# openclimatefix/graph_weather

Measured on AMD Instinct MI355X. Metric: forward forecasts/sec (1° grid, 102→78 feat), higher is better.
Workload: dtype f32; 1 GPU; c2: GraphWeatherForecaster 1deg grid (64800 nodes), 102->78 feat, batch=2 on rank 0, fp32, mesh res 2 (5882 nodes), random-init weights; global_batch=2, parallelism=batch-sharded x1, no collective in forward

## Files before the change

### graph_weather_amd/_lib.py

```python
from __future__ import annotations

import ctypes
import os
import subprocess
from ctypes import POINTER, Structure, c_char_p, c_float, c_int, c_int32, c_int64, c_size_t, c_void_p

_HERE = os.path.dirname(os.path.abspath(__file__))
CSRC = os.path.join(_HERE, "csrc")
LIB_PATH = os.path.join(CSRC, "libgw_amd.so")
HIPCC_FLAGS = ["--offload-arch=gfx950", "-O3", "-std=c++17", "-munsafe-fp-atomics", "-shared", "-fPIC"]

ABI_VERSION = 19
DTYPE_F32, DTYPE_BF16, DTYPE_BF16X3 = 0, 1, 2
LAYOUT_ROWS_F32, LAYOUT_EDGE_TILES_BF16, LAYOUT_ROWS_F16, LAYOUT_ROWS_BF16K = 0, 1, 2, 3
EDGE_DETERMINISTIC, EDGE_SEGMENT_TILES, EDGE_AGG_BF16K, EDGE_SEGMENT_SPLIT = 1, 2, 4, 8

EXPORTS = [
    "gw_version", "gw_last_error", "gw_debug_timestamps", "gw_packed_floats", "gw_pack_linear", "gw_packed_bytes_bf16",
    "gw_pack_linear_bf16", "gw_packed_bytes_bf16x3", "gw_pack_linear_bf16x3", "gw_padded_n", "gw_pad_vector", "gw_pack_many", "gw_mlp_chain_backward", "gw_mlp_chain_backward_bf16x3", "gw_mlp_ln_chain_backward",
    "gw_mlp_forward", "gw_mlp_post_forward", "gw_project_forward", "gw_edge_update_forward", "gw_edge_update_workspace_bytes", "gw_edge_tiles_bytes",
    "gw_edge_rows_to_tiles", "gw_node_update_forward", "gw_node_update_row_split_groups", "gw_node_update_head_forward",
    "gw_normalized_mse_forward", "gw_gemm_f32", "gw_relu_backward", "gw_layernorm_backward", "gw_gather_rows",
    "gw_segment_sum_rows", "gw_normalized_mse_backward", "gw_adamw_step", "gw_nudging_forward", "gw_nudging_backward",
    "gw_linear_forward", "gw_linear_gather_forward", "gw_layernorm_forward", "gw_add_rows", "gw_gather_rows_wide", "gw_segment_sum_rows_wide",
    "gw_constraint_workspace_bytes", "gw_constraint_forward", "gw_constraint_backward",
    "gw_thermal_conv_forward", "gw_thermal_conv_wgrad_workspace_bytes", "gw_thermal_conv_wgrad", "gw_thermal_colsum_workspace_bytes",
    "gw_thermal_colsum", "gw_thermal_groupnorm_workspace_bytes", "gw_thermal_groupnorm_forward", "gw_thermal_groupnorm_backward",
    "gw_thermal_maxpool_forward", "gw_thermal_maxpool_backward", "gw_thermal_resize_forward", "gw_thermal_resize_backward",
    "gw_thermal_rows",
    "gw_amse_mmax", "gw_amse_dft_rows", "gw_amse_legendre_floats", "gw_amse_coeff_floats", "gw_amse_workspace_bytes",
    "gw_amse_forward", "gw_amse_backward",
    "gw_modulate_workspace_bytes", "gw_sdl_forward", "gw_sdl_backward", "gw_film_forward", "gw_film_backward",
    "gw_attention_forward", "gw_attention_backward", "gw_knn_interpolate_forward", "gw_knn_interpolate_backward",
    "gw_gelu_forward", "gw_gelu_backward",
    "gw_attention_axial_forward", "gw_attention_axial_backward",
    "gw_patch_workspace_bytes", "gw_patch_embed_forward", "gw_patch_embed_backward", "gw_patch_expand_forward",
    "gw_patch_expand_backward",
    "gw_attention_masked_forward", "gw_attention_masked_backward",
    "gw_earth_loss_workspace_bytes", "gw_earth_loss_forward", "gw_earth_loss_backward",
    "gw_token_mean_forward", "gw_token_mean_backward", "gw_relu_forward", "gw_row_scale",
    "gw_conv3d_workspace_bytes", "gw_conv3d_forward", "gw_conv3d_backward",
    "gw_gemm_tn_ordered_workspace_bytes", "gw_gemm_tn_ordered", "gw_layernorm_backward_ordered_workspace_bytes",
    "gw_layernorm_backward_ordered",
]

GEMM_NN, GEMM_TN, GEMM_TN_BF16X3 = 0, 1, 2


class GwOperand(Structure):
    _fields_ = [("ptr", c_void_p), ("index", c_void_p), ("rows_per_batch", c_int32), ("ld", c_int32), ("k", c_int32),
                ("projected", c_int32), ("layout", c_int32)]


class GwMlpWeights(Structure):
    _fields_ = [("w1", c_void_p * 3), ("b1", c_void_p), ("w_mid", c_void_p), ("b_mid", c_void_p), ("w_out", c_void_p),
                ("b_out", c_void_p), ("ln_gamma", c_void_p), ("ln_beta", c_void_p), ("hidden", c_int32),
                ("n_mid", c_int32), ("n_out", c_int32), ("weight_dtype", c_int32), ("ln_width", c_int32), ("k_in", c_int32),
                ("out_rows", c_int32)]


PACK_MAX_ITEMS = 16


class GwPackItem(Structure):
    _fields_ = [("w", c_void_p), ("stride_f", c_int64), ("stride_k", c_int64), ("n_out", c_int32), ("kseg", c_int32),
                ("rows", c_int32), ("reserved", c_int32), ("out", c_void_p)]
# ... 96 lines not shown
    L.gw_pad_vector.argtypes = [c_void_p, c_int, c_void_p, c_void_p]
    L.gw_mlp_chain_backward.restype = c_int
    L.gw_mlp_chain_backward.argtypes = [c_int64, c_void_p, c_int32, c_int32, POINTER(c_void_p), POINTER(c_void_p), POINTER(c_void_p),
                                        c_int32, POINTER(c_void_p), POINTER(c_void_p), c_void_p]
    L.gw_mlp_chain_backward_bf16x3.restype = c_int
    L.gw_mlp_chain_backward_bf16x3.argtypes = L.gw_mlp_chain_backward.argtypes
    L.gw_mlp_ln_chain_backward.restype = c_int
    L.gw_mlp_ln_chain_backward.argtypes = [c_int32, c_int64, c_void_p, c_int32, c_void_p, c_int32, c_int32, c_void_p, c_int32,
                                           c_void_p, c_void_p, c_void_p, c_void_p, c_void_p,
                                           c_int32, POINTER(c_void_p), POINTER(c_void_p), POINTER(c_void_p), c_void_p,
                                           c_int32, POINTER(c_void_p), POINTER(c_void_p), POINTER(c_void_p), c_int32, ctypes.c_uint32, c_void_p]
    L.gw_pack_many.restype = c_int
    L.gw_pack_many.argtypes = [c_int32, c_int32, POINTER(GwPackItem), c_int32, POINTER(GwPadItem), c_void_p]
    L.gw_mlp_forward.restype = c_int
    L.gw_mlp_forward.argtypes = [c_int64, c_int32, POINTER(GwOperand), POINTER(GwMlpWeights), POINTER(GwOperand),
                                 c_void_p, c_int32, POINTER(GwActivationSave), c_void_p]
    L.gw_mlp_post_forward.restype = c_int
    L.gw_mlp_post_forward.argtypes = [c_int64, c_int32, POINTER(GwOperand), POINTER(GwMlpWeights), c_void_p, c_int32, c_int32,
                                      POINTER(c_void_p), POINTER(c_void_p), c_int32, c_void_p]
    L.gw_edge_update_forward.restype = c_int
    L.gw_edge_update_forward.argtypes = [c_int32, c_int32, c_void_p, c_void_p, POINTER(GwOperand), POINTER(GwOperand),
                                         POINTER(GwOperand), POINTER(GwOperand), POINTER(GwMlpWeights), c_void_p, c_int32, c_void_p,
                                         c_int32, POINTER(GwActivationSave), c_void_p, c_size_t, c_int32, c_void_p]
    L.gw_edge_tiles_bytes.restype = c_size_t
    L.gw_edge_tiles_bytes.argtypes = [c_int32, c_int32]
    L.gw_edge_rows_to_tiles.restype = c_int
    L.gw_edge_rows_to_tiles.argtypes = [c_int32, c_int32, c_void_p, c_int32, c_int32, c_void_p, c_void_p]
    L.gw_edge_update_workspace_bytes.restype = c_size_t
    L.gw_edge_update_workspace_bytes.argtypes = [c_int32, c_int32, POINTER(GwOperand), POINTER(GwOperand), POINTER(GwOperand),
                                                 POINTER(GwMlpWeights), c_int32]
    L.gw_node_update_forward.restype = c_int
    L.gw_node_update_forward.argtypes = [c_int64, c_int32, POINTER(GwOperand), POINTER(GwOperand), POINTER(GwOperand),
                                         POINTER(GwMlpWeights), c_void_p, c_int32, POINTER(GwActivationSave), c_int32,
                                         POINTER(c_void_p), POINTER(c_void_p), c_int32, c_void_p, c_void_p]
    L.gw_node_update_row_split_groups.restype = c_int
    L.gw_node_update_row_split_groups.argtypes = [c_int64]
    L.gw_node_update_head_forward.restype = c_int
    L.gw_node_update_head_forward.argtypes = [c_int64, c_int32, POINTER(GwOperand), POINTER(GwOperand), POINTER(GwMlpWeights),
                                              POINTER(GwMlpWeights), POINTER(GwOperand), c_void_p, c_int32, c_void_p]
    L.gw_project_forward.restype = c_int
    L.gw_project_forward.argtypes = [c_int64, c_int32, POINTER(GwOperand), c_int32, POINTER(c_void_p), POINTER(c_void_p),
                                     c_int32, c_int32, c_int32, c_void_p, c_void_p, c_void_p]
    L.gw_normalized_mse_forward.restype = c_int
    L.gw_normalized_mse_forward.argtypes = [c_void_p, c_void_p, c_void_p, c_int32, c_void_p, c_int32, c_int32, c_int32, c_int32,
                                            c_void_p, c_void_p]
    L.gw_gemm_f32.restype = c_int
# ... 194 lines not shown
```

### graph_weather_amd/autograd.py

```python
from __future__ import annotations

from typing import List, Optional, Sequence, Tuple

import torch

from . import _lib, ops
from .ops import Operand, SavedActivations


def _st(t: torch.Tensor) -> int:
    return torch.cuda.current_stream(t.device).cuda_stream


def _L():
    return _lib.lib()


def gemm_nn(a: torch.Tensor, b: torch.Tensor, n: int, b_col0: int = 0, out: Optional[torch.Tensor] = None) -> torch.Tensor:
    m, k = int(a.shape[0]), int(a.shape[1])
    if out is None:
        out = torch.empty((m, n), dtype=torch.float32, device=a.device)
    _lib.check(_L().gw_gemm_f32(_lib.GEMM_NN, m, n, k, a.data_ptr(), int(a.stride(0)), b.data_ptr() + 4 * b_col0,
                                int(b.stride(0)), out.data_ptr(), int(out.stride(0)), None, _st(a)), "gw_gemm_f32 NN")
    return out
# ... 274 lines not shown
        grads[0] = gW0
        dx = fo[fan[0]] if fan else None
        dres = None
        if ctx.has_res and ctx.needs_input_grad[2]:
            n_out = int(dy.shape[1])
            if res.shape[1] == n_out:
                dres = dy
            else:
                dres = torch.zeros_like(res)
                dres[:, :n_out] = dy
        return (None, dx, dres, None, None, None, None, *grads)


def mlp_rows(mlp, x2: torch.Tensor, n_rows: int, rows_per_batch: int, residual_op: Optional[Operand] = None) -> torch.Tensor:
    params = mlp.native_params()
    if residual_op is None:
        return MLPRowsFunction.apply(mlp, x2, None, 0, 0, n_rows, rows_per_batch, *params)
    return MLPRowsFunction.apply(mlp, x2, residual_op.tensor, residual_op.rows_per_batch, residual_op.k, n_rows, rows_per_batch,
                                 *params)


class RecomputeFunction(torch.autograd.Function):

    @staticmethod
    def forward(ctx, fn, n_in, params, *tensors):
        ctx.fn, ctx.n_in, ctx.params = fn, n_in, params
        ctx.save_for_backward(*tensors[:n_in])
        with torch.no_grad():
            outs = fn(*tensors[:n_in])
        return tuple(outs)

    @staticmethod
    def backward(ctx, *douts):
        n_in, params = ctx.n_in, ctx.params
        ins = [t.detach().requires_grad_(bool(need)) for t, need in zip(ctx.saved_tensors, ctx.needs_input_grad[3:3 + n_in])]
        with torch.enable_grad():
            outs = ctx.fn(*ins)
        pairs = [(o, d) for o, d in zip(outs, douts) if d is not None and o.requires_grad]
        wanted = [t for t in ins if t.requires_grad] + [p for p in params if p.requires_grad]
        got = iter(torch.autograd.grad([o for o, _ in pairs], wanted, [d for _, d in pairs], allow_unused=True)) if pairs and wanted \
            else iter(())
        g_in = [next(got, None) if t.requires_grad else None for t in ins]
        g_par = [next(got, None) if p.requires_grad else None for p in params]
        return (None, None, None, *g_in, *g_par)


def recompute(fn, inputs: Sequence[torch.Tensor], module) -> Tuple[torch.Tensor, ...]:
    mods = module if isinstance(module, (list, tuple)) else [module]
    params = [p for m in mods for p in m.parameters()]
    if not torch.is_grad_enabled() or not (any(p.requires_grad for p in params) or any(t.requires_grad for t in inputs)):
        return tuple(fn(*inputs))
    return RecomputeFunction.apply(fn, len(inputs), params, *inputs, *params)


def _input_grad_joined(mlp, d: torch.Tensor, W: torch.Tensor, lo: int, hi: int, addend: Optional[torch.Tensor]) -> torch.Tensor:
    if addend is None:
        return input_grad(mlp, 0, d, W, lo, hi)
    pt = _packed_transposed(mlp, 0, W, lo, hi) if (d.shape[1] == 256 and d.stride(0) % 4 == 0 and d.shape[0] > 0) else None
    if (pt is not None and addend.shape == d.shape and addend.stride(1) == 1 and addend.stride(0) % 4 == 0 and addend.stride(0) >= 256
            and addend.dtype == torch.float32):
        out = torch.empty((int(d.shape[0]), 256), dtype=torch.float32, device=d.device)
        chain_backward(d, [], [(pt, out)], fan_add=[addend])
        return out
    return input_grad(mlp, 0, d, W, lo, hi).add_(addend)


class ProjectFunction(torch.autograd.Function):
# ... 264 lines not shown
```

### graph_weather_amd/layers.py

```python
from __future__ import annotations

from typing import List, Optional, Tuple

import torch
from torch import nn

from . import autograd as ag
from . import ops
from . import routes
from . import wide
from .autograd import OperandSpec
from .graphs import ForecastGraphs, GraphPlan, build_forecast_graphs
from .ops import BF16X3, Operand, PackedMLP
from .thermalizer import ThermalizerLayer

_NORMS = ["LayerNorm", "GraphNorm", "InstanceNorm", "BatchNorm", "MessageNorm"]


def _ver(t: torch.Tensor) -> int:
    return -1 if t.is_inference() else t._version


def _version_key(params) -> tuple:
    return tuple((p.data_ptr(), _ver(p), p.device) for p in params)
# ... 600 lines not shown

    def mesh_embedding(self) -> torch.Tensor:
        ps = list(self.node_encoder.parameters()) + [self.h3_nodes]
        return self._cached("mesh", ps, lambda: self.node_encoder.table(self.h3_nodes if _autograd_on(self) else self.h3_nodes.detach()))

    def encoder_edge_embedding(self, plan: GraphPlan) -> torch.Tensor:
        return self._cached("enc_e", list(self.edge_encoder.parameters()), lambda: self.edge_encoder.table(plan.edge_attr))

    def latent_edge_embedding(self, plan: GraphPlan) -> torch.Tensor:
        return self._cached("lat_e", list(self.latent_edge_encoder.parameters()),
                            lambda: self.latent_edge_encoder.table(plan.edge_attr))

    def encode(self, features: torch.Tensor, post_w=None):
        if features.dim() != 3 or features.shape[1] != self.num_latlons:
            raise RuntimeError("features must be [B, %d, input_dim]" % self.num_latlons)
        B, G, F = (int(s) for s in features.shape)
        if wide.encoder_is_wide(self):
            return wide.encode(self, features)
        feats = features.contiguous().reshape(B * G, F)
        enc_plan, _ = self._plans(features.device)
        team = self.team_path(features)
        x3 = self.split_path(features)
        ne = self.node_encoder
        fused_ps = None
        if ((team and ne.compute_dtype == torch.bfloat16) or (x3 and ne.compute_dtype == BF16X3)) and not ne._layout()[4] \
                and 32 < ne.native_k() <= 128:
            pm_e0 = self.graph_processor.blocks[0].edge_model.edge_mlp.packed()
            k = ne.native_k()
            x2 = feats if k <= F else torch.nn.functional.pad(feats, (0, k - F))
            fused_ps = ops.mlp_post_forward(ne.packed(), Operand(x2, G, k), B * G, G, [pm_e0.w1[0]], post_half=team)[1][0]
            xg = None
        else:
            xg = ne.run(feats, B * G, G)
        xm = self.mesh_embedding()
        e = self.encoder_edge_embedding(enc_plan)
        blk = self.graph_processor.blocks[0]
        _check_native_dims(*self.graph_processor._dims)
        pd_xm, pe, px_xm, e = self._static_projections(blk, xm, e)
        x_src, e_res = Feed(xg, G, "raw"), e
        seg = None
        if team or x3:
            pm_e = blk.edge_model.edge_mlp.packed()
            if fused_ps is None:
                fused_ps = ops.project_forward([pm_e.w1[0]], Operand(xg, G, 256), B * G, G, out_half=team)[0]
            x_src = Feed(fused_ps, G, "proj")
            px_xm = self._team_node_product(blk, enc_plan, e, px_xm)
            e_res = None
        if team:
            seg = enc_plan.seg_tiles(split=True)
            if seg is not None:
                pe = self._cached("enc_pe_pad", list(self.parameters()), lambda: seg.pad_rows(pe))
        if post_w is not None:
            x, _, posts, agg0 = blk.run(B, enc_plan, x_src, Feed(pd_xm, 0, "proj"), Feed(pe, 0, "proj"), e_res, 0,
                                        Feed(px_xm, 0, "proj"), xm, 0, False, features.device, tag="encoder_edge",
                                        post_w=post_w, post_zero=True, seg=seg)
            return x, posts, agg0
        x, _ = blk.run(B, enc_plan, x_src, Feed(pd_xm, 0, "proj"), Feed(pe, 0, "proj"), e_res, 0,
                       Feed(px_xm, 0, "proj"), xm, 0, False, features.device, tag="encoder_edge", seg=seg)
        return x

    def team_path(self, features: Optional[torch.Tensor] = None) -> bool:
        return self._block_route(features) == routes.BLOCK_TEAM

    def _block_route(self, features: Optional[torch.Tensor] = None) -> str:
        blk = self.graph_processor.blocks[0]
        mlp_e, mlp_n = blk.edge_model.edge_mlp, blk.node_model.node_mlp
        is_wide = wide.encoder_is_wide(self)
        auto = False if is_wide else _autograd_on(self, features)
        if is_wide or auto:
            return routes.BLOCK_ROWS
        return routes.block_route(_form(mlp_e), mlp_n.compute_dtype, self.graphs.enc_plan.num_edges, False, False,
                                  bool(blk.deterministic))

    def split_path(self, features: Optional[torch.Tensor] = None) -> bool:
        return self._block_route(features) == routes.BLOCK_SPLIT

    def _team_node_product(self, blk, plan: GraphPlan, e: torch.Tensor, px_xm: torch.Tensor) -> torch.Tensor:
        def make():
            pm_n = blk.node_model.node_mlp.packed()
            n_e = int(e.shape[0])
            e_sum = ag.segment_sum_rows(e, n_e, 1, 1, plan.n_dst, plan.dst_ptr(), None)
            pa = ops.project_forward([pm_n.w1[1]], Operand(e_sum, plan.n_dst, 256), plan.n_dst, plan.n_dst)[0]
# ... 352 lines not shown
```

### graph_weather_amd/ops.py

```python
from __future__ import annotations

from dataclasses import dataclass
from typing import List, Optional, Sequence, Tuple

import torch

from . import _lib
from ._lib import GwActivationSave, GwMlpWeights, GwOperand


class KernelTimer:

    def __init__(self, tags):
        self.tags = set(tags)
        self.events = {t: [] for t in self.tags}
        self.units = {t: [] for t in self.tags}

    def start(self, tag):
        if tag not in self.tags:
            return None
        ev = (torch.cuda.Event(enable_timing=True), torch.cuda.Event(enable_timing=True))
        ev[0].record()
        return ev

    def stop(self, tag, ev, units: int = 1):
        if ev is not None:
            ev[1].record()
            self.events[tag].append(ev)
            self.units[tag].append(int(units))

    def mean_units(self, tag) -> float:
        u = self.units[tag]
        return sum(u) / max(1, len(u))

    def mean_ms(self, tag) -> float:
        evs = self.events[tag]
        return sum(a.elapsed_time(b) for a, b in evs) / max(1, len(evs))


TIMER: Optional[KernelTimer] = None

EDGE_STREAM = True
"""float32 inference: the decoder's edge update runs without the per-edge residual on the decoder-form kernel of
csrc/gw_edge_stream.hip (the segment sums of the batch-shared edge embedding enter the node update as a cached product).
``False`` forces the per-edge residual route on ``edge_kernel`` (csrc/gw_edge.hip).  Read on every ``decode``."""


def _stream(t: torch.Tensor) -> int:
    return torch.cuda.current_stream(t.device).cuda_stream


class _NoGuard:
    def __enter__(self):
        return None

    def __exit__(self, *exc):
        return False


_NO_GUARD = _NoGuard()


def on_device_of(t: torch.Tensor):
    idx = t.device.index
    if idx is None or idx == torch.cuda.current_device():
        return _NO_GUARD
    return torch.cuda.device(idx)

# ... 281 lines not shown
            _require(e_out, "e_out")
    n_edges = int(src.shape[0])
    wc = pm.c((x_src.k > 0 and not x_src.projected, x_dst.k > 0 and not x_dst.projected, e_in.k > 0 and not e_in.projected))
    xs, xd, ei = x_src.c(), x_dst.c(), e_in.c()
    flags = _lib.EDGE_DETERMINISTIC if deterministic else 0
    if segment_tiles:
        flags |= _lib.EDGE_SEGMENT_TILES | (_lib.EDGE_AGG_BF16K if agg_bf16 else 0) | (_lib.EDGE_SEGMENT_SPLIT if segment_split else 0)
    ws, ws_bytes = None, 0
    if save is None:
        ws_bytes = int(_lib.lib().gw_edge_update_workspace_bytes(batch, n_edges, xs, xd, ei, wc, flags))
        if ws_bytes:
            ws = torch.empty(ws_bytes, dtype=torch.uint8, device=agg.device)
    ev = TIMER.start(tag) if TIMER is not None else None
    with on_device_of(agg):
        _lib.check(_lib.lib().gw_edge_update_forward(batch, n_edges, src.data_ptr(), dst.data_ptr(), xs, xd, ei,
                                                     e_res.c(), wc, None if e_out is None else e_out.data_ptr(), e_out_layout,
                                                     agg.data_ptr(), n_dst, None if save is None else save.c(),
                                                     None if ws is None else ws.data_ptr(), ws_bytes, flags, _stream(agg)),
                   "gw_edge_update_forward")
    if ev is not None:
        TIMER.stop(tag, ev, batch)


def node_update_forward(pm: PackedMLP, n_rows: int, rows_per_batch: int, x: Operand, x_res: Operand, agg: Operand,
                        out: Optional[torch.Tensor] = None, save: Optional[SavedActivations] = None,
                        post_w: Optional[Sequence[torch.Tensor]] = None, zero_rows: Optional[torch.Tensor] = None,
                        post_half: bool = False):
    import ctypes

    dev = agg.tensor.device
    if out is None:
        out = torch.empty((n_rows, pm.n_out), dtype=torch.float32, device=dev)
    _require(out, "out")
    wc = pm.c((x.k > 0 and not x.projected, True, False))
    n_post = 0 if post_w is None else len(post_w)
    outs, wp, op = [], None, None
    if n_post:
        outs = [torch.empty((n_rows, 256), dtype=torch.float16 if post_half else torch.float32, device=dev) for _ in range(n_post)]
        wp = (ctypes.c_void_p * n_post)(*[w_.data_ptr() for w_ in post_w])
        op = (ctypes.c_void_p * n_post)(*[o_.data_ptr() for o_ in outs])
    with on_device_of(out):
        _lib.check(_lib.lib().gw_node_update_forward(n_rows, rows_per_batch, x.c(), x_res.c(), agg.c(), wc, out.data_ptr(),
                                                     int(out.stride(0)), None if save is None else save.c(), n_post, wp, op,
                                                     _lib.LAYOUT_ROWS_F16 if (post_half and n_post) else _lib.LAYOUT_ROWS_F32,
                                                     None if zero_rows is None else zero_rows.data_ptr(), _stream(out)),
                   "gw_node_update_forward")
# ... 200 lines not shown
```

### graph_weather_amd/routes.py

```python
from __future__ import annotations

from dataclasses import dataclass
from typing import Optional, Sequence, Tuple

import torch

BF16X3 = "bf16x3"



@dataclass(frozen=True)
class MlpForm:

    dtype: object
    n_mid: int
    ln_width: int
    has_norm: bool

    @staticmethod
    def of(mlp, packed=None) -> "MlpForm":
        pm = mlp.packed() if packed is None else packed
        return MlpForm(mlp.compute_dtype, int(pm.n_mid), int(pm.ln_width), pm.gamma is not None)


# ... 31 lines not shown

BLOCK_ROWS = "rows"
BLOCK_TEAM = "team"
BLOCK_SPLIT = "split"


def block_route(edge: MlpForm, node_dtype, n_edges: int, wide: bool, autograd: bool, deterministic: bool) -> str:
    if wide or autograd or n_edges <= 0:
        return BLOCK_ROWS
    if edge.dtype == BF16X3 and node_dtype == BF16X3:
        return BLOCK_SPLIT
    if edge.dtype == torch.bfloat16 and node_dtype == torch.bfloat16 and not deterministic and resident_bf16(edge, n_edges):
        return BLOCK_TEAM
    return BLOCK_ROWS


def decoder_stream(edge: MlpForm, node_dtype, n_edges: int, wide: bool, autograd: bool, deterministic: bool, enabled: bool) -> bool:
    if not enabled or wide or autograd or deterministic or n_edges <= 0:
        return False
    return (edge.dtype == torch.float32 and node_dtype == torch.float32 and edge.n_mid == 1 and edge.ln_width == 0
            and edge.has_norm)




def stack_on_segment_tiles(blocks: Sequence[Tuple[MlpForm, object, bool]], n_edges: int, max_slots: Optional[int]) -> bool:
    if len(blocks) == 0 or n_edges <= 0 or max_slots is None or max_slots > 16:
        return False
    return all(resident_bf16(e, n_edges) and nd == torch.bfloat16 and not det for e, nd, det in blocks)


def segment_route_allowed(train: bool, want_edges: bool, lo: int, shared: bool) -> bool:
    return (not train) and (not want_edges) and lo == 0 and shared


def mesh_streams(streams_attr: int, edge_dtypes: Sequence[object], batch: int) -> int:
    if streams_attr > 0:
        return max(1, min(int(streams_attr), batch))
    tiled = all(d in (torch.float32, BF16X3) for d in edge_dtypes)
    return 2 if (tiled and batch >= 2) else 1



NODE_COLS64 = "cols64"


# ... 13 lines not shown
```

### include/gw_amd.h

```cpp
#ifndef GW_AMD_H
#define GW_AMD_H

#include <stddef.h>
#include <stdint.h>

#ifdef __cplusplus
extern "C" {
#endif

#define GW_OK 0
#define GW_E_BADARG (-1)
#define GW_E_UNSUPPORTED (-2)
#define GW_E_LAUNCH (-3)

#define GW_ABI_VERSION 19

#define GW_DTYPE_F32 0
#define GW_DTYPE_BF16 1
#define GW_DTYPE_BF16X3 2

#define GW_LAYOUT_ROWS_F32 0
#define GW_LAYOUT_EDGE_TILES_BF16 1
#define GW_LAYOUT_ROWS_F16 2
#define GW_LAYOUT_ROWS_BF16K 3
// ... 87 lines not shown
                             const void* const* fan_w, float* const* fan_out, const float* const* fan_add, int32_t fan_add_ld,
                             uint32_t fan_add_dn_mask, void* stream);

int gw_project_forward(int64_t n_rows, int32_t rows_per_batch, const gw_operand* x, int32_t n_slices,
                       const float* const* w_slices, void* const* outs, int32_t out_ld,
                       int32_t out_layout ,
                       int32_t weight_dtype ,
                       const float* relu_mask ,
                       float* zero_rows ,
                       void* stream);

int gw_edge_update_forward(int32_t batch, int32_t n_edges, const int32_t* src, const int32_t* dst,
                           const gw_operand* x_src, const gw_operand* x_dst, const gw_operand* e_in,
                           const gw_operand* e_res, const gw_mlp_weights* w,
                           void* e_out ,
                           int32_t e_out_layout , float* agg ,
                           int32_t n_dst, const struct gw_activation_save* save ,
                           void* workspace , size_t workspace_bytes, int32_t flags , void* stream);
size_t gw_edge_tiles_bytes(int32_t batch, int32_t n_edges);
int gw_edge_rows_to_tiles(int32_t batch, int32_t n_edges, const float* rows, int32_t rows_per_batch, int32_t ld, void* tiles,
                          void* stream);
size_t gw_edge_update_workspace_bytes(int32_t batch, int32_t n_edges, const gw_operand* x_src, const gw_operand* x_dst,
                                      const gw_operand* e_in, const gw_mlp_weights* w, int32_t flags);

int gw_node_update_forward(int64_t n_rows, int32_t rows_per_batch, const gw_operand* x, const gw_operand* x_res,
                           const gw_operand* agg, const gw_mlp_weights* w, float* x_out, int32_t out_ld,
                           const struct gw_activation_save* save ,
                           int32_t n_post , const float* const* post_w, void* const* post_out,
                           int32_t post_layout ,
                           float* zero_rows , void* stream);

int gw_node_update_row_split_groups(int64_t n_rows);

int gw_node_update_head_forward(int64_t n_rows, int32_t rows_per_batch, const gw_operand* x, const gw_operand* agg,
                                const gw_mlp_weights* w, const gw_mlp_weights* head, const gw_operand* residual ,
                                float* out, int32_t out_ld, void* stream);

int gw_normalized_mse_forward(const float* pred, const float* target,
                              const float* inv_var ,
                              int32_t inv_var_full, const float* lat_weights, int32_t num_unique_lat, int32_t batch, int32_t nodes,
                              int32_t channels, float* loss_out, void* stream);


typedef struct gw_activation_save {
  float* hidden;
  int64_t hidden_stride;
// ... 223 lines not shown
```

Baseline: 312.6 forecasts/s.

## Fuse encoder node MLP and edge update into one kernel launch

Adds a HIP kernel that runs the node encoder MLP (with LayerNorm) on each grid row in registers and feeds the result directly into the encoder edge-update MLP with scatter aggregation. This avoids writing the encoded grid rows to global memory and reading them back, and drops one launch. The team node product can also run on a side stream overlapping the fused kernel. In exchange there is a large, register-heavy kernel with a narrow routing condition (fp32 inference, edges equal to latlons), and register pressure could limit occupancy.

```diff
diff --git a/graph_weather_amd/_lib.py b/graph_weather_amd/_lib.py
--- a/graph_weather_amd/_lib.py
+++ b/graph_weather_amd/_lib.py
@@ -42,6 +42,7 @@
     "gw_conv3d_workspace_bytes", "gw_conv3d_forward", "gw_conv3d_backward",
     "gw_gemm_tn_ordered_workspace_bytes", "gw_gemm_tn_ordered", "gw_layernorm_backward_ordered_workspace_bytes",
     "gw_layernorm_backward_ordered",
+    "gw_encoder_fused_forward",
 ]
 
 GEMM_NN, GEMM_TN, GEMM_TN_BF16X3 = 0, 1, 2
@@ -184,6 +185,10 @@
     L.gw_edge_update_forward.argtypes = [c_int32, c_int32, c_void_p, c_void_p, POINTER(GwOperand), POINTER(GwOperand),
                                          POINTER(GwOperand), POINTER(GwOperand), POINTER(GwMlpWeights), c_void_p, c_int32, c_void_p,
                                          c_int32, POINTER(GwActivationSave), c_void_p, c_size_t, c_int32, c_void_p]
+    L.gw_encoder_fused_forward.restype = c_int
+    L.gw_encoder_fused_forward.argtypes = [c_int32, c_int32, c_void_p, c_void_p, POINTER(GwOperand), POINTER(GwMlpWeights),
+                                           POINTER(GwOperand), POINTER(GwOperand), POINTER(GwOperand), POINTER(GwMlpWeights), c_void_p,
+                                           c_int32, POINTER(GwActivationSave), c_int32, c_void_p]
     L.gw_edge_tiles_bytes.restype = c_size_t
     L.gw_edge_tiles_bytes.argtypes = [c_int32, c_int32]
     L.gw_edge_rows_to_tiles.restype = c_int
diff --git a/graph_weather_amd/autograd.py b/graph_weather_amd/autograd.py
--- a/graph_weather_amd/autograd.py
+++ b/graph_weather_amd/autograd.py
@@ -320,12 +320,18 @@
 
 class RecomputeFunction(torch.autograd.Function):
 
+    first_pass_depth = 0
+
     @staticmethod
     def forward(ctx, fn, n_in, params, *tensors):
         ctx.fn, ctx.n_in, ctx.params = fn, n_in, params
         ctx.save_for_backward(*tensors[:n_in])
-        with torch.no_grad():
-            outs = fn(*tensors[:n_in])
+        RecomputeFunction.first_pass_depth += 1
+        try:
+            with torch.no_grad():
+                outs = fn(*tensors[:n_in])
+        finally:
+            RecomputeFunction.first_pass_depth -= 1
         return tuple(outs)
 
     @staticmethod
@@ -341,6 +347,10 @@
         g_in = [next(got, None) if t.requires_grad else None for t in ins]
         g_par = [next(got, None) if p.requires_grad else None for p in params]
         return (None, None, None, *g_in, *g_par)
+
+
+def in_recomputed_first_pass() -> bool:
+    return RecomputeFunction.first_pass_depth > 0
 
 
 def recompute(fn, inputs: Sequence[torch.Tensor], module) -> Tuple[torch.Tensor, ...]:
diff --git a/graph_weather_amd/csrc/gw_encoder_fused.hip b/graph_weather_amd/csrc/gw_encoder_fused.hip
--- /dev/null
+++ b/graph_weather_amd/csrc/gw_encoder_fused.hip
@@ -0,0 +1,565 @@
+
+#include <hip/hip_runtime.h>
+#include <stdint.h>
+#include <string.h>
+
+#include "gw_device.hpp"
+#include "gw_edge_common.hpp"
+#include "gw_internal.hpp"
+
+using namespace gw;
+
+namespace {
+
+constexpr int kNodeSteps = 28;
+constexpr int kConstFloats = 10 * 256;
+constexpr int kConstOff = kStageFloats + kColsPerWG;
+constexpr int kEncfLdsBytes = (kConstOff + kConstFloats) * 4;
+static_assert(kEncfLdsBytes == 77056, "staging (66 560) + destination ids (256) + constants (10 240)");
+static_assert((kConstOff * 4) % 16 == 0, "constants are read as 16-byte vectors");
+static_assert(2 * kEncfLdsBytes <= 160 * 1024, "two workgroups per CU must fit the 160 KiB of LDS");
+constexpr int kB1 = 0, kBMid = 256, kBOut = 512, kGamma = 768, kBeta = 1024;
+constexpr int kNodeSet = 0, kEdgeSet = 1280;
+
+struct EncfArgs {
+  int n_cols;
+  int n_edges;
+  int n_dst;
+  int stagger;
+  int xcd_base;
+  int xcd_rem;
+  const int* src;
+  const int* dst;
+  const float* feat;
+  int feat_rows_pb;
+  int feat_ld;
+  int k_valid;
+  const float* n_w1;
+  const float* n_w_mid;
+  const float* n_w_out;
+  const float* n_const[5];
+  const float* w_raw;
+  const float* w_mid;
+  const float* w_out;
+  const float* e_const[5];
+  const float* p_ptr[2];
+  int p_rows_pb[2];
+  int p_ld[2];
+  int p_kind[2];
+  const float* res_ptr;
+  int res_rows_pb;
+  int res_ld;
+  float* agg;
+};
+
+constexpr int kChunksPerTile = 4 + 5 * kChunksPerLayer;
+
+__device__ __forceinline__ const float* chunk_src(const EncfArgs& a, int i) {
+  if (i < 4) return a.n_w1 + (size_t)i * kChunkFloats;
+  i -= 4;
+  const float* m = i < 8 ? a.n_w_mid : (i < 16 ? a.n_w_out : (i < 24 ? a.w_raw : (i < 32 ? a.w_mid : a.w_out)));
+  return m + (size_t)(i & 7) * kChunkFloats;
+}
+
+__device__ __forceinline__ float hld1(const float* p) {
+  float v;
+  asm volatile("global_load_dword %0, %1, off" : "=v"(v) : "v"(p) : "memory");
+  return v;
+}
+typedef float f32x2 __attribute__((ext_vector_type(2)));
+__device__ __forceinline__ f32x2 hld2(const float* p) {
+  f32x2 v;
+  asm volatile("global_load_dwordx2 %0, %1, off" : "=v"(v) : "v"(p) : "memory");
+  return v;
+}
+__device__ __forceinline__ void wait_const(float (&c)[10]) {
+  asm volatile("s_waitcnt vmcnt(0)"
+               : "+v"(c[0]), "+v"(c[1]), "+v"(c[2]), "+v"(c[3]), "+v"(c[4]), "+v"(c[5]), "+v"(c[6]), "+v"(c[7]), "+v"(c[8]), "+v"(c[9])
+               :
+               : "memory");
+}
+__device__ __forceinline__ void wait_pairs(f32x2 (&r)[14]) {
+  asm volatile("s_waitcnt vmcnt(0)"
+               : "+v"(r[0]), "+v"(r[1]), "+v"(r[2]), "+v"(r[3]), "+v"(r[4]), "+v"(r[5]), "+v"(r[6]), "+v"(r[7]), "+v"(r[8]), "+v"(r[9]),
+                 "+v"(r[10]), "+v"(r[11]), "+v"(r[12]), "+v"(r[13])
+               :
+               : "memory");
+}
+__device__ __forceinline__ void wait_singles(float (&r)[kNodeSteps]) {
+  asm volatile("s_waitcnt vmcnt(0)"
+               : "+v"(r[0]), "+v"(r[1]), "+v"(r[2]), "+v"(r[3]), "+v"(r[4]), "+v"(r[5]), "+v"(r[6]), "+v"(r[7]), "+v"(r[8]), "+v"(r[9]),
+                 "+v"(r[10]), "+v"(r[11]), "+v"(r[12]), "+v"(r[13])
+               :
+               : "memory");
+  asm volatile("s_waitcnt vmcnt(0)"
+               : "+v"(r[14]), "+v"(r[15]), "+v"(r[16]), "+v"(r[17]), "+v"(r[18]), "+v"(r[19]), "+v"(r[20]), "+v"(r[21]), "+v"(r[22]),
+                 "+v"(r[23]), "+v"(r[24]), "+v"(r[25]), "+v"(r[26]), "+v"(r[27])
+               :
+               : "memory");
+}
+
+#define GW_FCHUNK(ACC, IN, OFF, NS, NP, DS, WAIT_STMT)                                                          \
+  {                                                                                                            \
+    const float* bl_ = lds + (ci & 1) * kLdsBufFloats + lane * 4;                                              \
+    const float* nsrc_ = chunk_src(a, (NP) > 0 ? ci + 1 : ci);                                                 \
+    _Pragma("unroll") for (int s_ = 0; s_ < (NS); ++s_) {                                                      \
+      f32x4 a_nxt_[4];                                                                                         \
+      if ((NP) > 0 && s_ < (DS))                                                                               \
+        issue_pieces<((NP) > 0 ? (NP) / (DS) : 1)>(nsrc_, ((ci + 1) & 1) * kLdsBufFloats, s_ * ((NP) / (DS)), lane, wave); \
+      if (s_ + 1 < (NS)) {                                                                                     \
+        _Pragma("unroll") for (int b4 = 0; b4 < 4; ++b4) a_nxt_[b4] = *(const f32x4*)(bl_ + (s_ + 1) * 1024 + b4 * 256); \
+      } else if ((NP) > 0) {                                                                                   \
+        WAIT_STMT;                                                                                             \
+        lds_barrier();                                                                                         \
+        const float* bn_ = lds + ((ci + 1) & 1) * kLdsBufFloats + lane * 4;                                    \
+        _Pragma("unroll") for (int b4 = 0; b4 < 4; ++b4) a_nxt_[b4] = *(const f32x4*)(bn_ + b4 * 256);          \
+      }                                                                                                        \
+      const float b_ = IN[(OFF) + s_];                                                                         \
+      __builtin_amdgcn_sched_barrier(0);                                                                       \
+      _Pragma("unroll") for (int t = 0; t < 16; ++t)                                                           \
+          ACC[t] = __builtin_amdgcn_mfma_f32_16x16x4f32(a_cur[t >> 2][t & 3], b_, ACC[t], 0, 0, 0);             \
+      __builtin_amdgcn_sched_barrier(0);                                                                       \
+      if (s_ + 1 < (NS) || (NP) > 0) {                                                                         \
+        _Pragma("unroll") for (int b4 = 0; b4 < 4; ++b4) a_cur[b4] = a_nxt_[b4];                                \
+      }                                                                                                        \
+    }                                                                                                          \
+    ++ci;                                                                                                      \
+  }
+
+template <bool RES, int NPROJ>
+__global__ __launch_bounds__(kThreads, 2) void encfused_kernel(const EncfArgs a) {
+  float* const lds = lds_base();
+  const float* const cst = lds + kConstOff;
+  const int lane = threadIdx.x & 63;
+  const int wave = __builtin_amdgcn_readfirstlane(threadIdx.x >> 6);
+  const int j = lane & 15;
+  const int q = lane >> 4;
+  int tile = blockIdx.x;
+  if (a.xcd_base > 0) {
+    const int xcd = tile & 7, idx = tile >> 3;
+    tile = xcd * a.xcd_base + (xcd < a.xcd_rem ? xcd : a.xcd_rem) + idx;
+  }
+  const int tile_c0 = tile * kColsPerWG;
+  const int c_raw = tile_c0 + wave * kColsPerWave + j;
+  const bool valid = c_raw < a.n_cols;
+  const int c = valid ? c_raw : a.n_cols - 1;
+  const int b = c / a.n_edges;
+  const int k = c - b * a.n_edges;
+
+  if (a.stagger > 0 && (blockIdx.x >> 8) == 1) {
+    for (int i = 0; i < a.stagger; ++i) __builtin_amdgcn_s_sleep(127);
+  }
+
+  int s_idx = hldi(a.src + k);
+  int d_idx = hldi(a.dst + k);
+  float cv[10];
+  {
+    const int f = threadIdx.x;
+#pragma unroll
+    for (int i = 0; i < 5; ++i) cv[i] = hld1(a.n_const[i] + f);
+#pragma unroll
+    for (int i = 0; i < 5; ++i) cv[5 + i] = hld1(a.e_const[i] + f);
+  }
+  issue_chunk32k(chunk_src(a, 0), lds, lane, wave);
+  int ci = 0;
+  wait_regs<18>(s_idx, d_idx);
+  const float* prow[NPROJ];
+#pragma unroll
+  for (int p = 0; p < NPROJ; ++p) {
+    const int r = a.p_kind[p] == 1 ? d_idx : k;
+    prow[p] = a.p_ptr[p] + ((size_t)b * (size_t)a.p_rows_pb[p] + (size_t)r) * (size_t)a.p_ld[p] + 4 * q;
+  }
+  int gd_id = valid ? b * a.n_dst + d_idx : -1;
+  asm volatile("" : "+v"(gd_id));
+
+  float x[kNodeSteps];
+  {
+    const float* row = a.feat + ((size_t)b * (size_t)a.feat_rows_pb + (size_t)s_idx) * (size_t)a.feat_ld;
+    const bool pairs = (a.k_valid & 1) == 0 && ((size_t)row & 7) == 0;
+    if (pairs) {
+      f32x2 pv[14];
+#pragma unroll
+      for (int i = 0; i < 7; ++i)
+#pragma unroll
+        for (int r = 0; r < 2; ++r) {
+          const int kk = 16 * i + 4 * q + 2 * r;
+          pv[2 * i + r] = hld2(row + (kk < a.k_valid ? kk : 0));
+        }
+      wait_pairs(pv);
+#pragma unroll
+      for (int i = 0; i < 7; ++i)
+#pragma unroll
+        for (int r = 0; r < 2; ++r) {
+          const bool in = 16 * i + 4 * q + 2 * r < a.k_valid;
+          x[4 * i + 2 * r] = in ? pv[2 * i + r].x : 0.f;
+          x[4 * i + 2 * r + 1] = in ? pv[2 * i + r].y : 0.f;
+        }
+    } else {
+#pragma unroll
+      for (int i = 0; i < 7; ++i)
+#pragma unroll
+        for (int r = 0; r < 4; ++r) {
+          const int kk = 16 * i + 4 * q + r;
+          x[4 * i + r] = hld1(row + (kk < a.k_valid ? kk : 0));
+        }
+      wait_singles(x);
+#pragma unroll
+      for (int i = 0; i < 7; ++i)
+#pragma unroll
+        for (int r = 0; r < 4; ++r)
+          if (!(16 * i + 4 * q + r < a.k_valid)) x[4 * i + r] = 0.f;
+    }
+  }
+  wait_const(cv);
+  {
+    float* cw = lds + kConstOff + threadIdx.x;
+#pragma unroll
+    for (int i = 0; i < 10; ++i) cw[256 * i] = cv[i];
+  }
+  lds_barrier();
+
+  f32x4 a_cur[4];
+#pragma unroll
+  for (int b4 = 0; b4 < 4; ++b4) a_cur[b4] = *(const f32x4*)(lds + lane * 4 + b4 * 256);
+
+  f32x4 o[16];
+  {
+    f32x4 acc[16];
+#pragma unroll
+    for (int t = 0; t < 16; ++t) acc[t] = *(const f32x4*)(cst + kNodeSet + kB1 + 16 * t + 4 * q);
+    GW_FCHUNK(acc, x, 0, 8, 8, 4, wait_vm<0>())
+    GW_FCHUNK(acc, x, 8, 8, 8, 4, wait_vm<0>())
+    GW_FCHUNK(acc, x, 16, 8, 4, 4, wait_vm<0>())
+    GW_FCHUNK(acc, x, 24, 4, 8, 2, wait_vm<0>())
+    f32x4 acc2[16];
+#pragma unroll
+    for (int t = 0; t < 16; ++t) acc2[t] = *(const f32x4*)(cst + kNodeSet + kBMid + 16 * t + 4 * q);
+#pragma unroll
+    for (int cc = 0; cc < kChunksPerLayer; ++cc) {
+      float in8[8];
+#pragma unroll
+      for (int r = 0; r < 4; ++r) {
+        in8[r] = fmaxf(acc[2 * cc][r], 0.f);
+        in8[4 + r] = fmaxf(acc[2 * cc + 1][r], 0.f);
+      }
+      GW_FCHUNK(acc2, in8, 0, 8, 8, 4, wait_vm<0>())
+    }
+    float hin[64];
+#pragma unroll
+    for (int t = 0; t < 16; ++t)
+#pragma unroll
+      for (int r = 0; r < 4; ++r) hin[4 * t + r] = fmaxf(acc2[t][r], 0.f);
+#pragma unroll
+    for (int t = 0; t < 16; ++t) o[t] = *(const f32x4*)(cst + kNodeSet + kBOut + 16 * t + 4 * q);
+#pragma unroll
+    for (int cc = 0; cc < kChunksPerLayer; ++cc) GW_FCHUNK(o, hin, 8 * cc, 8, 8, 4, wait_vm<0>())
+    constexpr float inv_n = 1.0f / 256.0f;
+    float s = 0.f;
+#pragma unroll
+    for (int t = 0; t < 16; ++t) s += (o[t].x + o[t].y) + (o[t].z + o[t].w);
+    s += __shfl_xor(s, 16);
+    s += __shfl_xor(s, 32);
+    const float mean = s * inv_n;
+    float v = 0.f;
+#pragma unroll
+    for (int t = 0; t < 16; ++t)
+#pragma unroll
+      for (int r = 0; r < 4; ++r) {
+        const float d = o[t][r] - mean;
+        v += d * d;
+      }
+    v += __shfl_xor(v, 16);
+    v += __shfl_xor(v, 32);
+    const float rstd = 1.0f / sqrtf(v * inv_n + 1e-5f);
+#pragma unroll
+    for (int t = 0; t < 16; ++t) {
+      const f32x4 gm = *(const f32x4*)(cst + kNodeSet + kGamma + 16 * t + 4 * q);
+      const f32x4 bt = *(const f32x4*)(cst + kNodeSet + kBeta + 16 * t + 4 * q);
+#pragma unroll
+      for (int r = 0; r < 4; ++r) o[t][r] = (o[t][r] - mean) * rstd * gm[r] + bt[r];
+    }
+  }
+
+  f32x4 ring[2][NPROJ][2];
+#define GW_REQUEST_SLICE(slot, slice)                                          \
+  {                                                                            \
+    _Pragma("unroll") for (int p = 0; p < NPROJ; ++p) {                        \
+      ring[slot][p][0] = hld4<128 * (slice)>(prow[p]);                         \
+      ring[slot][p][1] = hld4<128 * (slice) + 64>(prow[p]);                    \
+    }                                                                          \
+  }
+#define GW_CONSUME_SLICE(slot, slice)                                          \
+  {                                                                            \
+    f32x4 v0_ = acc[2 * (slice)] + ring[slot][0][0];                           \
+    f32x4 v1_ = acc[2 * (slice) + 1] + ring[slot][0][1];                       \
+    _Pragma("unroll") for (int p = 1; p < NPROJ; ++p) {                        \
+      v0_ += ring[slot][p][0];                                                 \
+      v1_ += ring[slot][p][1];                                                 \
+    }                                                                          \
+    _Pragma("unroll") for (int r = 0; r < 4; ++r) {                            \
+      in8[r] = fmaxf(v0_[r], 0.f);                                             \
+      in8[4 + r] = fmaxf(v1_[r], 0.f);                                         \
+    }                                                                          \
+  }
+
+  f32x4 acc[16];
+  f32x4 acc2[16];
+  float in8[8];
+  {
+#pragma unroll
+    for (int t = 0; t < 16; ++t) acc[t] = *(const f32x4*)(cst + kEdgeSet + kB1 + 16 * t + 4 * q);
+    float xr[64];
+#pragma unroll
+    for (int i = 0; i < 16; ++i) {
+      xr[4 * i + 0] = o[i].x;
+      xr[4 * i + 1] = o[i].y;
+      xr[4 * i + 2] = o[i].z;
+      xr[4 * i + 3] = o[i].w;
+    }
+#pragma unroll
+    for (int cc = 0; cc < kChunksPerLayer; ++cc) {
+      if (cc == kChunksPerLayer - 3) {
+        GW_REQUEST_SLICE(0, 0)
+        GW_REQUEST_SLICE(1, 1)
+      }
+      if (cc == kChunksPerLayer - 1) {
+#pragma unroll
+        for (int t = 0; t < 16; ++t) acc2[t] = *(const f32x4*)(cst + kEdgeSet + kBMid + 16 * t + 4 * q);
+      }
+      GW_FCHUNK(acc, xr, 8 * cc, 8, 8, 4, wait_vm<0>())
+    }
+    wait_regs<0>(ring[0]);
+    wait_regs<0>(ring[1]);
+    GW_CONSUME_SLICE(0, 0)
+    GW_REQUEST_SLICE(0, 2)
+  }
+
+#define GW_PRODUCE_CHUNK(cc)                                                              \
+  {                                                                                       \
+    if ((cc) <= 6) {                                                                      \
+      GW_FCHUNK(acc2, in8, 0, 8, 8, 4, wait_regs<0>(ring[((cc) + 1) & 1]))                 \
+    } else {                                                                              \
+      GW_FCHUNK(acc2, in8, 0, 8, 8, 4, wait_vm<0>())                                       \
+    }                                                                                     \
+    if ((cc) + 1 < kChunksPerLayer) GW_CONSUME_SLICE(((cc) + 1) & 1, (cc) + 1)             \
+  }
+  GW_PRODUCE_CHUNK(0)
+  GW_REQUEST_SLICE(1, 3)
+  GW_PRODUCE_CHUNK(1)
+  GW_REQUEST_SLICE(0, 4)
+  GW_PRODUCE_CHUNK(2)
+  GW_REQUEST_SLICE(1, 5)
+  GW_PRODUCE_CHUNK(3)
+  GW_REQUEST_SLICE(0, 6)
+  GW_PRODUCE_CHUNK(4)
+  GW_REQUEST_SLICE(1, 7)
+  GW_PRODUCE_CHUNK(5)
+  GW_PRODUCE_CHUNK(6)
+  GW_PRODUCE_CHUNK(7)
+
+  float hin[64];
+#pragma unroll
+  for (int t = 0; t < 16; ++t)
+#pragma unroll
+    for (int r = 0; r < 4; ++r) hin[4 * t + r] = fmaxf(acc2[t][r], 0.f);
+  f32x4 rres[16];
+#pragma unroll
+  for (int t = 0; t < 16; ++t) o[t] = f32x4{0.f, 0.f, 0.f, 0.f};
+#pragma unroll
+  for (int cc = 0; cc < kChunksPerLayer; ++cc) {
+    if (cc + 1 < kChunksPerLayer) {
+      GW_FCHUNK(o, hin, 8 * cc, 8, 8, 4, wait_vm<0>())
+    } else {
+      GW_FCHUNK(o, hin, 8 * cc, 8, 0, 1, wait_vm<0>())
+    }
+    if (RES && (cc == 3 || cc == 5)) {
+      const float* rrow = a.res_ptr + ((size_t)b * (size_t)a.res_rows_pb + (size_t)k) * (size_t)a.res_ld + 4 * q;
+      if (cc == 3) hld_half_row<0>(rres, rrow); else hld_half_row<1>(rres, rrow);
+    }
+  }
+  if (RES) wait_regs<0>(rres);
+
+  {
+#pragma unroll
+    for (int t = 0; t < 16; ++t) o[t] += *(const f32x4*)(cst + kEdgeSet + kBOut + 16 * t + 4 * q);
+    constexpr float inv_n = 1.0f / 256.0f;
+    float s = 0.f;
+#pragma unroll
+    for (int t = 0; t < 16; ++t) s += (o[t].x + o[t].y) + (o[t].z + o[t].w);
+    s += __shfl_xor(s, 16);
+    s += __shfl_xor(s, 32);
+    const float mean = s * inv_n;
+    float v = 0.f;
+#pragma unroll
+    for (int t = 0; t < 16; ++t)
+#pragma unroll
+      for (int r = 0; r < 4; ++r) {
+        const float d = o[t][r] - mean;
+        v += d * d;
+      }
+    v += __shfl_xor(v, 16);
+    v += __shfl_xor(v, 32);
+    const float rstd = 1.0f / sqrtf(v * inv_n + 1e-5f);
+#pragma unroll
+    for (int t = 0; t < 16; ++t) {
+      const f32x4 gm = *(const f32x4*)(cst + kEdgeSet + kGamma + 16 * t + 4 * q);
+      const f32x4 bt = *(const f32x4*)(cst + kEdgeSet + kBeta + 16 * t + 4 * q);
+#pragma unroll
+      for (int r = 0; r < 4; ++r) {
+        if (RES) o[t][r] = (o[t][r] - mean) * rstd * gm[r] + bt[r] + rres[t][r];
+        else o[t][r] = (o[t][r] - mean) * rstd * gm[r] + bt[r];
+      }
+    }
+  }
+
+  __syncthreads();
+  {
+    float* srow = lds + (wave * kColsPerWave + j) * kStageLd + 4 * q;
+#pragma unroll
+    for (int t = 0; t < 16; ++t) *(f32x4*)(srow + 16 * t) = o[t];
+    if (q == 0) ((int*)(lds + kStageFloats))[wave * kColsPerWave + j] = gd_id;
+  }
+  __syncthreads();
+  const int* gdl = (const int*)(lds + kStageFloats);
+
+  {
+    const int f = threadIdx.x;
+    float vv[kColsPerWG];
+#pragma unroll
+    for (int i = 0; i < kColsPerWG; ++i) vv[i] = lds[i * kStageLd + f];
+    const int gdv = gdl[lane];
+    const int gdn = gdl[lane < kColsPerWG - 1 ? lane + 1 : lane];
+    const unsigned long long ends = __ballot(lane == kColsPerWG - 1 || gdn != gdv);
+    float run = 0.f;
+    bool first = true;
+#pragma unroll
+    for (int i = 0; i < kColsPerWG; ++i) {
+      run += vv[i];
+      if (__builtin_expect((ends >> i) & 1ull, 0)) {
+        const int cur = __builtin_amdgcn_readlane(gdv, i);
+        if (cur >= 0) {
+          float* dstp = a.agg + (size_t)cur * 256 + f;
+          if (first || i == kColsPerWG - 1) {
+            __hip_atomic_fetch_add((GW_AS1 float*)dstp, run, __ATOMIC_RELAXED, __HIP_MEMORY_SCOPE_AGENT);
+          } else {
+            stg1(dstp, run);
+          }
+        }
+        first = false;
+        run = 0.f;
+      }
+    }
+  }
+#undef GW_REQUEST_SLICE
+#undef GW_CONSUME_SLICE
+#undef GW_PRODUCE_CHUNK
+}
+
+template <typename K>
+int launch(K kernel, const EncfArgs& a, void* stream) {
+  static DeviceOnce once;
+  if (once.first()) (void)hipFuncSetAttribute((const void*)kernel, hipFuncAttributeMaxDynamicSharedMemorySize, kEncfLdsBytes);
+  const int grid = (a.n_cols + kColsPerWG - 1) / kColsPerWG;
+  hipLaunchKernelGGL(kernel, dim3(grid), dim3(kThreads), kEncfLdsBytes, (hipStream_t)stream, a);
+  return check_launch("encfused_kernel launch");
+}
+
+inline bool node_encoder_ok(const gw_mlp_weights* w) {
+  return w->weight_dtype == GW_DTYPE_F32 && w->n_mid == 1 && w->hidden == 256 && w->n_out == 256 && w->w1[0] && w->b1 && w->w_mid &&
+         w->b_mid && w->w_out && w->b_out && w->ln_gamma && w->ln_beta && (w->ln_width == 0 || w->ln_width == 256);
+}
+
+}
+
+int gw_encoder_fused_forward(int32_t batch, int32_t n_edges, const int32_t* src, const int32_t* dst, const gw_operand* features,
+                             const gw_mlp_weights* w_node, const gw_operand* x_dst, const gw_operand* e_in, const gw_operand* e_res,
+                             const gw_mlp_weights* w_edge, float* agg, int32_t n_dst, const gw_activation_save* save, int32_t flags,
+                             void* stream) {
+  if (batch <= 0 || n_edges < 0 || n_dst <= 0 || !features || !w_node || !x_dst || !e_in || !e_res || !w_edge)
+    return set_error(GW_E_BADARG, "gw_encoder_fused_forward: bad arguments");
+  if (n_edges == 0) return GW_OK;
+  if (!src || !dst || !agg || !features->ptr) return set_error(GW_E_BADARG, "gw_encoder_fused_forward: bad arguments");
+  if ((int64_t)batch * n_edges >= (int64_t)1 << 31 || (int64_t)batch * n_dst >= (int64_t)1 << 31)
+    return set_error(GW_E_UNSUPPORTED, "gw_encoder_fused_forward: batch*edges exceeds int32");
+  if (save || flags != 0)
+    return set_error(GW_E_UNSUPPORTED, "gw_encoder_fused_forward: inference in atomics mode on row tiles only (no activation saves, "
+                                       "no deterministic sums, no segment tiles)");
+  if (!node_encoder_ok(w_node) || features->layout != GW_LAYOUT_ROWS_F32 || features->projected || features->index ||
+      features->k <= 16 || features->k > 112 || features->ld < features->k || features->rows_per_batch <= 0 ||
+      (w_node->k_in > 0 && w_node->k_in != features->k))
+    return set_error(GW_E_UNSUPPORTED, "gw_encoder_fused_forward: float32 node encoder with one middle layer, widths 256, LayerNorm "
+                                       "over 256 and 17..112 input features as fp32 rows");
+  gw_operand raw;
+  memset(&raw, 0, sizeof(raw));
+  raw.ptr = features->ptr;
+  raw.rows_per_batch = features->rows_per_batch;
+  raw.ld = 256;
+  raw.k = 256;
+  raw.layout = GW_LAYOUT_ROWS_F32;
+  const gw_operand* pops[2] = {x_dst, e_in};
+  EncfArgs a;
+  memset(&a, 0, sizeof(a));
+  int n_proj = 0;
+  for (int i = 0; i < 2; ++i) {
+    if (pops[i]->k == 0) continue;
+    if (!pops[i]->projected || pops[i]->layout != GW_LAYOUT_ROWS_F32 || pops[i]->k != 256 || pops[i]->ld % 4 != 0 || !pops[i]->ptr)
+      return set_error(GW_E_UNSUPPORTED, "gw_encoder_fused_forward: x_dst / e_in are projected 256-wide fp32 rows (or k = 0)");
+    a.p_ptr[n_proj] = pops[i]->ptr;
+    a.p_rows_pb[n_proj] = pops[i]->rows_per_batch;
+    a.p_ld[n_proj] = pops[i]->ld;
+    a.p_kind[n_proj] = i + 1;
+    ++n_proj;
+  }
+  if (w_edge->hidden != 256 || w_edge->n_out != 256 || !w_edge->b1 || !w_edge->w_out || !w_edge->b_out || !w_edge->w1[0] || n_proj == 0 ||
+      !gw::edge_lds_eligible(&raw, x_dst, e_in, w_edge))
+    return set_error(GW_E_UNSUPPORTED, "gw_encoder_fused_forward: float32 edge MLP with one middle layer, widths 256, LayerNorm over "
+                                       "256, its x_src slice packed and one or two projected operands");
+  const bool res = e_res->k != 0;
+  if (res && (e_res->k != 256 || e_res->ld % 4 != 0 || !e_res->ptr || e_res->layout != GW_LAYOUT_ROWS_F32))
+    return set_error(GW_E_UNSUPPORTED, "gw_encoder_fused_forward: e_res (residual edge features) must be 256-wide fp32 rows (or k = 0)");
+  a.n_cols = batch * n_edges;
+  a.n_edges = n_edges;
+  a.n_dst = n_dst;
+  a.src = src;
+  a.dst = dst;
+  a.feat = features->ptr;
+  a.feat_rows_pb = features->rows_per_batch;
+  a.feat_ld = features->ld;
+  a.k_valid = features->k;
+  a.n_w1 = w_node->w1[0];
+  a.n_w_mid = w_node->w_mid;
+  a.n_w_out = w_node->w_out;
+  a.n_const[0] = w_node->b1;
+  a.n_const[1] = w_node->b_mid;
+  a.n_const[2] = w_node->b_out;
+  a.n_const[3] = w_node->ln_gamma;
+  a.n_const[4] = w_node->ln_beta;
+  a.w_raw = w_edge->w1[0];
+  a.w_mid = w_edge->w_mid;
+  a.w_out = w_edge->w_out;
+  a.e_const[0] = w_edge->b1;
+  a.e_const[1] = w_edge->b_mid;
+  a.e_const[2] = w_edge->b_out;
+  a.e_const[3] = w_edge->ln_gamma;
+  a.e_const[4] = w_edge->ln_beta;
+  if (res) {
+    a.res_ptr = e_res->ptr;
+    a.res_rows_pb = e_res->rows_per_batch;
+    a.res_ld = e_res->ld;
+  }
+  a.agg = agg;
+  const int tiles = (a.n_cols + kColsPerWG - 1) / kColsPerWG;
+  {
+    static const int stagger_override = GW_TUNE("GW_STAGGER", -1);
+    const int passes = 6;
+    a.stagger = stagger_override >= 0 ? stagger_override * passes : 2 * passes + 2;
+    if (tiles <= 256) a.stagger = 0;
+  }
+  {
+    static const int xcd_map = GW_TUNE("GW_XCD_MAP", 1);
+    a.xcd_base = (xcd_map != 0 && tiles >= 64) ? tiles / 8 : 0;
+    a.xcd_rem = tiles % 8;
+  }
+  if (res) return n_proj == 1 ? launch(encfused_kernel<true, 1>, a, stream) : launch(encfused_kernel<true, 2>, a, stream);
+  return n_proj == 1 ? launch(encfused_kernel<false, 1>, a, stream) : launch(encfused_kernel<false, 2>, a, stream);
+}
diff --git a/graph_weather_amd/layers.py b/graph_weather_amd/layers.py
--- a/graph_weather_amd/layers.py
+++ b/graph_weather_amd/layers.py
@@ -646,6 +646,7 @@
         team = self.team_path(features)
         x3 = self.split_path(features)
         ne = self.node_encoder
+        fused = F == ne.native_k() and self.fused_path(features)
         fused_ps = None
         if ((team and ne.compute_dtype == torch.bfloat16) or (x3 and ne.compute_dtype == BF16X3)) and not ne._layout()[4] \
                 and 32 < ne.native_k() <= 128:
@@ -653,6 +654,8 @@
             k = ne.native_k()
             x2 = feats if k <= F else torch.nn.functional.pad(feats, (0, k - F))
             fused_ps = ops.mlp_post_forward(ne.packed(), Operand(x2, G, k), B * G, G, [pm_e0.w1[0]], post_half=team)[1][0]
+            xg = None
+        elif fused:
             xg = None
         else:
             xg = ne.run(feats, B * G, G)
@@ -674,6 +677,31 @@
             seg = enc_plan.seg_tiles(split=True)
             if seg is not None:
                 pe = self._cached("enc_pe_pad", list(self.parameters()), lambda: seg.pad_rows(pe))
+        if fused:
+            dev = features.device
+            agg = torch.zeros((B * enc_plan.n_dst, 256), dtype=torch.float32, device=dev)
+            side = None
+            if not self._cache.fresh("enc_proj_team", _version_key(list(self.parameters()))):
+                main, side = torch.cuda.current_stream(dev), device_stream(dev, "mesh", 0)
+                side.wait_stream(main)
+            ops.encoder_fused_forward(ne.packed(), blk.edge_model.edge_mlp.packed(), B, enc_plan.src, enc_plan.dst,
+                                      Operand(feats, G, F), Operand(pd_xm, 0, 256, projected=True),
+                                      Operand(pe, 0, 256, projected=True), ops.ZERO, enc_plan.n_dst, agg, tag="encoder_edge")
+            if side is not None:
+                with torch.cuda.stream(side):
+                    px_xm = self._team_node_product(blk, enc_plan, e, px_xm)
+                px_xm.record_stream(main)
+                main.wait_stream(side)
+            else:
+                px_xm = self._team_node_product(blk, enc_plan, e, px_xm)
+            pm_n = blk.node_model.node_mlp.packed()
+            n_rows, n_dst = B * enc_plan.n_dst, enc_plan.n_dst
+            x_op, res_x, agg_op = Operand(px_xm, 0, 256, projected=True), Operand(xm, 0, 256), Operand(agg, n_dst, 256)
+            if post_w is not None:
+                agg0 = torch.empty((n_rows, 256), dtype=torch.float32, device=dev)
+                x, posts = ops.node_update_forward(pm_n, n_rows, n_dst, x_op, res_x, agg_op, post_w=post_w, zero_rows=agg0)
+                return x, posts, agg0
+            return ops.node_update_forward(pm_n, n_rows, n_dst, x_op, res_x, agg_op)
         if post_w is not None:
             x, _, posts, agg0 = blk.run(B, enc_plan, x_src, Feed(pd_xm, 0, "proj"), Feed(pe, 0, "proj"), e_res, 0,
                                         Feed(px_xm, 0, "proj"), xm, 0, False, features.device, tag="encoder_edge",
@@ -682,6 +710,20 @@
         x, _ = blk.run(B, enc_plan, x_src, Feed(pd_xm, 0, "proj"), Feed(pe, 0, "proj"), e_res, 0,
                        Feed(px_xm, 0, "proj"), xm, 0, False, features.device, tag="encoder_edge", seg=seg)
         return x
+
+    def fused_path(self, features: Optional[torch.Tensor] = None) -> bool:
+        blk = self.graph_processor.blocks[0]
+        ne, mlp_e, mlp_n = self.node_encoder, blk.edge_model.edge_mlp, blk.node_model.node_mlp
+        if wide.encoder_is_wide(self) or ne.compute_dtype != torch.float32 or mlp_e.compute_dtype != torch.float32:
+            return False
+
+        def form(m):
+            native = not m._layout()[4] and m._norm() is not None and len(m._linears()) == 3
+            return routes.MlpForm(torch.float32, 1 if native else -1, 0 if native else -1, native)
+
+        train = _autograd_on(self, features) or ag.in_recomputed_first_pass()
+        return routes.encoder_fused(form(ne), ne.native_k(), form(mlp_e), mlp_n.compute_dtype, self.graphs.enc_plan.num_edges,
+                                    self.num_latlons, False, train, bool(blk.deterministic), bool(ops.ENCODER_FUSED))
 
     def team_path(self, features: Optional[torch.Tensor] = None) -> bool:
         return self._block_route(features) == routes.BLOCK_TEAM
diff --git a/graph_weather_amd/ops.py b/graph_weather_amd/ops.py
--- a/graph_weather_amd/ops.py
+++ b/graph_weather_amd/ops.py
@@ -44,6 +44,11 @@
 """float32 inference: the decoder's edge update runs without the per-edge residual on the decoder-form kernel of
 csrc/gw_edge_stream.hip (the segment sums of the batch-shared edge embedding enter the node update as a cached product).
 ``False`` forces the per-edge residual route on ``edge_kernel`` (csrc/gw_edge.hip).  Read on every ``decode``."""
+
+ENCODER_FUSED = True
+"""float32 inference: the encoder's node encoder and edge update run as ONE launch (csrc/gw_encoder_fused.hip) that keeps the
+grid rows in registers and adds no per-edge residual (the segment sums of the batch-shared edge embedding enter the node update
+as a cached product).  ``False`` keeps the two launches (``chain_kernel`` + ``elds_kernel``).  Read on every ``encode``."""
 
 
 def _stream(t: torch.Tensor) -> int:
@@ -371,6 +376,26 @@
         TIMER.stop(tag, ev, batch)
 
 
+def encoder_fused_forward(pm_node: PackedMLP, pm_edge: PackedMLP, batch: int, src: torch.Tensor, dst: torch.Tensor,
+                          features: Operand, x_dst: Operand, e_in: Operand, e_res: Operand, n_dst: int, agg: torch.Tensor,
+                          tag: Optional[str] = None, save: Optional[SavedActivations] = None, deterministic: bool = False) -> None:
+    _require(src, "src", torch.int32)
+    _require(dst, "dst", torch.int32)
+    _require(agg, "agg")
+    n_edges = int(src.shape[0])
+    wn = pm_node.c()
+    we = pm_edge.c((True, False, False))
+    ev = TIMER.start(tag) if TIMER is not None else None
+    with on_device_of(agg):
+        _lib.check(_lib.lib().gw_encoder_fused_forward(batch, n_edges, src.data_ptr(), dst.data_ptr(), features.c(), wn, x_dst.c(),
+                                                       e_in.c(), e_res.c(), we, agg.data_ptr(), n_dst,
+                                                       None if save is None else save.c(),
+                                                       _lib.EDGE_DETERMINISTIC if deterministic else 0, _stream(agg)),
+                   "gw_encoder_fused_forward")
+    if ev is not None:
+        TIMER.stop(tag, ev, batch)
+
+
 def node_update_forward(pm: PackedMLP, n_rows: int, rows_per_batch: int, x: Operand, x_res: Operand, agg: Operand,
                         out: Optional[torch.Tensor] = None, save: Optional[SavedActivations] = None,
                         post_w: Optional[Sequence[torch.Tensor]] = None, zero_rows: Optional[torch.Tensor] = None,
diff --git a/graph_weather_amd/routes.py b/graph_weather_amd/routes.py
--- a/graph_weather_amd/routes.py
+++ b/graph_weather_amd/routes.py
@@ -77,6 +77,17 @@
             and edge.has_norm)
 
 
+def encoder_fused(node_enc: MlpForm, node_enc_k: int, edge: MlpForm, node_dtype, n_edges: int, num_latlons: int, wide: bool,
+                  autograd: bool, deterministic: bool, enabled: bool) -> bool:
+    if not enabled or wide or autograd or deterministic or n_edges <= 0 or n_edges != num_latlons:
+        return False
+    if not (node_enc.dtype == torch.float32 and node_enc.n_mid == 1 and node_enc.ln_width == 0 and node_enc.has_norm
+            and 16 < node_enc_k <= 112):
+        return False
+    return (edge.dtype == torch.float32 and node_dtype == torch.float32 and edge.n_mid == 1 and edge.ln_width == 0
+            and edge.has_norm)
+
+
 
 
 def stack_on_segment_tiles(blocks: Sequence[Tuple[MlpForm, object, bool]], n_edges: int, max_slots: Optional[int]) -> bool:
diff --git a/include/gw_amd.h b/include/gw_amd.h
--- a/include/gw_amd.h
+++ b/include/gw_amd.h
@@ -133,6 +133,11 @@
                           void* stream);
 size_t gw_edge_update_workspace_bytes(int32_t batch, int32_t n_edges, const gw_operand* x_src, const gw_operand* x_dst,
                                       const gw_operand* e_in, const gw_mlp_weights* w, int32_t flags);
+
+int gw_encoder_fused_forward(int32_t batch, int32_t n_edges, const int32_t* src, const int32_t* dst, const gw_operand* features,
+                             const gw_mlp_weights* w_node, const gw_operand* x_dst, const gw_operand* e_in, const gw_operand* e_res,
+                             const gw_mlp_weights* w_edge, float* agg , int32_t n_dst,
+                             const struct gw_activation_save* save , int32_t flags , void* stream);
 
 int gw_node_update_forward(int64_t n_rows, int32_t rows_per_batch, const gw_operand* x, const gw_operand* x_res,
                            const gw_operand* agg, const gw_mlp_weights* w, float* x_out, int32_t out_ld,
```

New measurement: 315.7 forecasts/s (median of 6 runs). 1.01x the previous value.
